# jyjblrd/Low-Cost-Mocap

Hardware: NVIDIA H100
Metric: mocap frame-sets/s (4-cam 640x480 synthetic, blob+epipolar+DLT) (higher is better)
Workload: dtype u8 pixels -> int64 moments -> f64 geometry

## Files before the change

### low-cost-mocap_b200/csrc/api.cu

```cuda
#include <stdarg.h>
#include <stdlib.h>
#include <math.h>
#include <new>
#include "common.cuh"
#include "camera_tables.h"

int blob_kernels_init(mocap_ctx* ctx);
int match_kernels_init(mocap_ctx* ctx);
int fused_kernel_init(mocap_ctx* ctx);
int tma_kernel_init(mocap_ctx* ctx);
int ba_dev_init(mocap_ctx* ctx);

int mocap_fail(mocap_ctx* ctx, int code, const char* fmt, ...) {
    if (ctx) {
        va_list ap;
        va_start(ap, fmt);
        vsnprintf(ctx->err, sizeof(ctx->err), fmt, ap);
        va_end(ap);
    }
    return code;
}

int ensure_scratch(mocap_ctx* ctx, size_t bytes) {
    if (bytes <= ctx->scratch_bytes) return MOCAP_OK;
// ... 28 lines not shown
    cfg->max_blobs = 32;
    cfg->max_segments = 1024;
    cfg->max_roots = 64;
    cfg->max_cands = 8;
    cfg->max_groups = 4096;
}

const char* mocap_last_error(const mocap_ctx* ctx) { return ctx ? ctx->err : "no context"; }

static bool is_pow2(int v) { return v > 0 && (v & (v - 1)) == 0; }

int mocap_create(mocap_ctx** out, const mocap_config* cfg) {
    if (!out || !cfg) return MOCAP_EINVAL;
    *out = nullptr;
    if (cfg->n_cam < 1 || cfg->n_cam > MOCAP_MAX_CAM || cfg->width < 16 || cfg->width % MOCAP_SEG_PX != 0 ||
        cfg->height < 1 || cfg->max_blobs < 1 || cfg->max_blobs > MOCAP_MAX_BLOBS ||
        !is_pow2(cfg->max_segments) || cfg->max_segments < 64 || cfg->max_segments > 4096 ||
        cfg->max_roots < 1 || cfg->max_roots > MOCAP_MAX_ROOTS || cfg->max_cands < 1 || cfg->max_cands > MOCAP_MAX_CANDS ||
        cfg->max_groups < 1 || (long long)cfg->width * cfg->height / MOCAP_SEG_PX > 65535)
        return MOCAP_EINVAL;
    int n_dev = 0;
    if (cudaGetDeviceCount(&n_dev) != cudaSuccess || n_dev <= 0 || cfg->device < 0 || cfg->device >= n_dev) {
        cudaGetLastError();
        return MOCAP_ENODEV;
    }
    cudaDeviceProp prop;
    if (cudaGetDeviceProperties(&prop, cfg->device) != cudaSuccess) return MOCAP_ENODEV;
    if (prop.major != 9 || prop.minor != 0) return MOCAP_ENODEV;
    if (cudaSetDevice(cfg->device) != cudaSuccess) return MOCAP_ENODEV;

    mocap_ctx* ctx = new (std::nothrow) mocap_ctx();
    if (!ctx) return MOCAP_ENOMEM;
    memset(ctx, 0, sizeof(*ctx));
    ctx->cfg = *cfg;
    ctx->num_sms = prop.multiProcessorCount;
    ctx->h_tables.n_cam = cfg->n_cam;
    int st = MOCAP_OK;
    do {
        if (cudaMalloc(&ctx->d_tables, sizeof(CameraTables)) != cudaSuccess) { st = MOCAP_ENOMEM; break; }
        if (cudaStreamCreateWithFlags(&ctx->copy_stream, cudaStreamNonBlocking) != cudaSuccess) { st = MOCAP_ECUDA; break; }
        if (cudaStreamCreateWithFlags(&ctx->copy_stream2, cudaStreamNonBlocking) != cudaSuccess) { st = MOCAP_ECUDA; break; }
        for (int k = 0; k < 2 * 64; ++k)
            if (cudaEventCreate(&ctx->tim_ev[k]) != cudaSuccess) { st = MOCAP_ECUDA; break; }
        if (st) break;
        for (int k = 0; k < 2; ++k) {
            if (cudaEventCreateWithFlags(&ctx->stage_free[k], cudaEventDisableTiming) != cudaSuccess) { st = MOCAP_ECUDA; break; }
            if (cudaEventCreateWithFlags(&ctx->copied[k], cudaEventDisableTiming) != cudaSuccess) { st = MOCAP_ECUDA; break; }
        }
        if (st) break;
        if ((st = blob_kernels_init(ctx)) != MOCAP_OK) break;
        if ((st = match_kernels_init(ctx)) != MOCAP_OK) break;
        {
            const char* mode = getenv("MOCAP_PIPELINE");
            ctx->use_fused = (mode && strcmp(mode, "split") == 0) ? 0 : 1;
            ctx->use_tma = (mode && strcmp(mode, "tma") == 0) ? 1 : 0;
            ctx->use_phased = (mode && strcmp(mode, "phased") == 0) ? 1 : 0;
            ctx->pipeline_auto = (mode && mode[0]) ? 0 : 1;
        }
        {
            void* h = nullptr;
            if (cudaHostAlloc(&h, 2 * sizeof(unsigned long long), cudaHostAllocMapped) != cudaSuccess) { st = MOCAP_ENOMEM; break; }
            memset(h, 0, 2 * sizeof(unsigned long long));
            ctx->h_stat = static_cast<volatile unsigned long long*>(h);
            void* d = nullptr;
            if (cudaHostGetDevicePointer(&d, h, 0) != cudaSuccess) { st = MOCAP_ECUDA; break; }
            ctx->d_stat_host = static_cast<unsigned long long*>(d);
            if (cudaMalloc(&ctx->d_stat_acc, sizeof(unsigned long long)) != cudaSuccess) { st = MOCAP_ENOMEM; break; }
            if (cudaMemset(ctx->d_stat_acc, 0, sizeof(unsigned long long)) != cudaSuccess) { st = MOCAP_ECUDA; break; }
        }
        if ((st = fused_kernel_init(ctx)) != MOCAP_OK) break;
        if ((st = tma_kernel_init(ctx)) != MOCAP_OK) break;
        if ((st = ba_dev_init(ctx)) != MOCAP_OK) break;
        if (ctx->tma_ctas_per_sm < 1) ctx->use_tma = 0;
    } while (0);
    if (st != MOCAP_OK) { mocap_destroy(ctx); return st; }
    *out = ctx;
    return MOCAP_OK;
}

void mocap_destroy(mocap_ctx* ctx) {
    if (!ctx) return;
    cudaSetDevice(ctx->cfg.device);
    cudaDeviceSynchronize();
    cudaFree(ctx->d_tables);
    cudaFree(ctx->d_seg_count); cudaFree(ctx->d_seg_list); cudaFree(ctx->d_worklist); cudaFree(ctx->d_work_count);
    cudaFree(ctx->d_set_worklist); cudaFree(ctx->d_img_done); cudaFree(ctx->d_set_done); cudaFree(ctx->d_unit_counter);
    cudaFree(ctx->d_blob_xy); cudaFree(ctx->d_blob_n); cudaFree(ctx->d_img_flags);
    cudaFree(ctx->d_stage[0]); cudaFree(ctx->d_stage[1]);
    cudaFree(ctx->d_obj); cudaFree(ctx->d_err); cudaFree(ctx->d_nobj); cudaFree(ctx->d_setflags);
    cudaFree(ctx->d_scratch);
    cudaFree(ctx->d_ba_ws);
    cudaFree(ctx->d_match_counter);
    cudaFree(ctx->d_match_items); cudaFree(ctx->d_match_partial); cudaFree(ctx->d_match_range); cudaFree(ctx->d_match_arrive);
    cudaFree(ctx->d_pp_m1); cudaFree(ctx->d_pp_m2); cudaFree(ctx->d_pp_rot);
    cudaFree(ctx->d_stat_acc);
    if (ctx->h_stat) cudaFreeHost(const_cast<unsigned long long*>(ctx->h_stat));
    if (ctx->copy_stream) cudaStreamDestroy(ctx->copy_stream);
    if (ctx->copy_stream2) cudaStreamDestroy(ctx->copy_stream2);
    for (int k = 0; k < 2 * 64; ++k) if (ctx->tim_ev[k]) cudaEventDestroy(ctx->tim_ev[k]);
    for (int k = 0; k < 2; ++k) if (ctx->stage_free[k]) cudaEventDestroy(ctx->stage_free[k]);
    for (int k = 0; k < 2; ++k) if (ctx->copied[k]) cudaEventDestroy(ctx->copied[k]);
    delete ctx;
}

int mocap_set_stream(mocap_ctx* ctx, void* cuda_stream) {
    if (!ctx) return MOCAP_EINVAL;
    ctx->stream = reinterpret_cast<cudaStream_t>(cuda_stream);
    return MOCAP_OK;
}

int mocap_set_cameras(mocap_ctx* ctx, const double* K, const double* R, const double* t) {
    if (!ctx || !K || !R || !t) return MOCAP_EINVAL;
    const int C = ctx->cfg.n_cam;
    CameraTables& T = ctx->h_tables;
    build_camera_tables(T, C, K, R, t);
    CUDA_TRY(ctx, cudaSetDevice(ctx->cfg.device));
    CUDA_TRY(ctx, cudaMemcpyAsync(ctx->d_tables, &T, sizeof(T), cudaMemcpyHostToDevice, ctx->stream));
    CUDA_TRY(ctx, cudaStreamSynchronize(ctx->stream));
    ctx->cameras_set = true;
    return MOCAP_OK;
}

int mocap_set_world_transform(mocap_ctx* ctx, const double* M) {
    if (!ctx) return MOCAP_EINVAL;
    CameraTables& T = ctx->h_tables;
    T.use_world = M ? 1 : 0;
    if (M) memcpy(T.world, M, 16 * sizeof(double));
    CUDA_TRY(ctx, cudaMemcpyAsync(ctx->d_tables, &T, sizeof(T), cudaMemcpyHostToDevice, ctx->stream));
    CUDA_TRY(ctx, cudaStreamSynchronize(ctx->stream));
    return MOCAP_OK;
}

static bool pick_fused(const mocap_ctx* ctx, int channels) {
    if (!ctx->use_fused) return false;
    if (channels != 1 && (ctx->use_tma || ctx->use_phased)) return false;
    if (!ctx->pipeline_auto) return true;
    const unsigned long long blobs = ctx->h_stat[0], images = ctx->h_stat[1];
    if (images == 0) return true;
    return (double)blobs * ctx->cfg.n_cam <= (double)MOCAP_HEAVY_BLOBS_PER_SET * (double)images;
}

static int ensure_images(mocap_ctx* ctx, int n_images) {
    if (n_images <= ctx->cap_images) return MOCAP_OK;
    CUDA_TRY(ctx, cudaStreamSynchronize(ctx->stream));
    cudaFree(ctx->d_seg_count); cudaFree(ctx->d_seg_list); cudaFree(ctx->d_worklist); cudaFree(ctx->d_work_count); cudaFree(ctx->d_set_worklist); cudaFree(ctx->d_img_done); cudaFree(ctx->d_set_done); cudaFree(ctx->d_unit_counter); cudaFree(ctx->d_blob_xy); cudaFree(ctx->d_blob_n); cudaFree(ctx->d_img_flags);
    ctx->d_seg_count = nullptr; ctx->d_seg_list = nullptr; ctx->d_worklist = nullptr; ctx->d_work_count = nullptr; ctx->d_set_worklist = nullptr; ctx->d_img_done = nullptr; ctx->d_set_done = nullptr; ctx->d_unit_counter = nullptr; ctx->d_blob_xy = nullptr; ctx->d_blob_n = nullptr; ctx->d_img_flags = nullptr;
    ctx->cap_images = 0;
    const size_t n = (size_t)n_images;
    CUDA_TRY(ctx, cudaMalloc(&ctx->d_seg_count, n * sizeof(uint32_t)));
    CUDA_TRY(ctx, cudaMalloc(&ctx->d_seg_list, n * ctx->cfg.max_segments * sizeof(uint32_t)));
    CUDA_TRY(ctx, cudaMalloc(&ctx->d_worklist, n * sizeof(uint32_t)));
    CUDA_TRY(ctx, cudaMalloc(&ctx->d_work_count, 4 * sizeof(uint32_t)));
    CUDA_TRY(ctx, cudaMemsetAsync(ctx->d_work_count, 0, 4 * sizeof(uint32_t), ctx->stream));
    CUDA_TRY(ctx, cudaMalloc(&ctx->d_set_worklist, n * sizeof(uint32_t)));
    CUDA_TRY(ctx, cudaMalloc(&ctx->d_img_done, n * sizeof(uint32_t)));
    CUDA_TRY(ctx, cudaMalloc(&ctx->d_set_done, 2 * n * sizeof(uint32_t)));
    CUDA_TRY(ctx, cudaMalloc(&ctx->d_unit_counter, sizeof(unsigned long long)));
    CUDA_TRY(ctx, cudaMemsetAsync(ctx->d_img_done, 0, n * sizeof(uint32_t), ctx->stream));
    CUDA_TRY(ctx, cudaMemsetAsync(ctx->d_set_done, 0, 2 * n * sizeof(uint32_t), ctx->stream));
    CUDA_TRY(ctx, cudaMalloc(&ctx->d_blob_xy, n * ctx->cfg.max_blobs * 2 * sizeof(int32_t)));
    CUDA_TRY(ctx, cudaMalloc(&ctx->d_blob_n, n * sizeof(int32_t)));
    CUDA_TRY(ctx, cudaMalloc(&ctx->d_img_flags, n * sizeof(int32_t)));
    CUDA_TRY(ctx, cudaMemsetAsync(ctx->d_seg_count, 0, n * sizeof(uint32_t), ctx->stream));
    ctx->cap_images = n_images;
    return MOCAP_OK;
}
// ... 239 lines not shown
```

### low-cost-mocap_b200/csrc/ba_dev.cu

```cuda
#include "common.cuh"
#include "ba_device.cuh"

#define BA_THREADS 512

__global__ void __launch_bounds__(BA_THREADS, 1) k_ba_solve(const BAParams P) {
    extern __shared__ __align__(16) unsigned char ba_smem_raw[];
    ba_solve_body(P, ba_smem_raw);
}

__global__ void __launch_bounds__(1024)
k_track_offsets(const int32_t* __restrict__ n_obj, const double* __restrict__ err, int n_sets, int RMAX, double max_err,
                int capacity, int32_t* __restrict__ offs, int32_t* __restrict__ n_points) {
    __shared__ int warp_sum[32];
    __shared__ int carry;
    const int tid = threadIdx.x, lane = tid & 31, wid = tid >> 5;
    if (tid == 0) carry = 0;
    __syncthreads();
    for (int s0 = 0; s0 < n_sets; s0 += blockDim.x) {
        const int s = s0 + tid;
        int kept = 0;
        if (s < n_sets) {
            const int k = min(n_obj[s], RMAX);
            if (max_err > 0.0) { for (int r = 0; r < k; ++r) kept += (err[(size_t)s * RMAX + r] <= max_err) ? 1 : 0; }
            else kept = k;
        }
        int v = kept;
#pragma unroll
        for (int o = 1; o < 32; o <<= 1) { const int u = __shfl_up_sync(0xffffffffu, v, o); if (lane >= o) v += u; }
        if (lane == 31) warp_sum[wid] = v;
        __syncthreads();
        if (wid == 0) {
            int w = lane < (int)(blockDim.x >> 5) ? warp_sum[lane] : 0;
#pragma unroll
            for (int o = 1; o < 32; o <<= 1) { const int u = __shfl_up_sync(0xffffffffu, w, o); if (lane >= o) w += u; }
            warp_sum[lane] = w;
        }
        __syncthreads();
        const int before = carry + (wid > 0 ? warp_sum[wid - 1] : 0) + v - kept;
        if (s < n_sets) offs[s] = before;
        __syncthreads();
        if (tid == (int)blockDim.x - 1) carry = before + kept;
        __syncthreads();
    }
    if (tid == 0) *n_points = carry < capacity ? carry : capacity;
}

__global__ void __launch_bounds__(256)
k_tracks_to_obs(const int32_t* __restrict__ track_xy, const int32_t* __restrict__ n_obj, const double* __restrict__ err,
                const int32_t* __restrict__ offs, int n_sets, int RMAX, int C, double max_err, int capacity,
                double* __restrict__ obs, uint8_t* __restrict__ mask) {
    const long long idx = (long long)blockIdx.x * blockDim.x + threadIdx.x;
    if (idx >= (long long)n_sets * RMAX) return;
    const int s = (int)(idx / RMAX), r = (int)(idx - (long long)s * RMAX);
    if (r >= min(n_obj[s], RMAX)) return;
    int rank = r;
    if (max_err > 0.0) {
        if (!(err[(size_t)s * RMAX + r] <= max_err)) return;
        rank = 0;
        for (int q = 0; q < r; ++q) rank += (err[(size_t)s * RMAX + q] <= max_err) ? 1 : 0;
    }
    const int p = offs[s] + rank;
    if (p >= capacity) return;
    const int32_t* t = track_xy + ((size_t)s * RMAX + r) * C * 2;
    for (int c = 0; c < C; ++c) {
        const int x = t[2 * c], y = t[2 * c + 1];
        const bool seen = x >= 0;
        obs[((size_t)p * C + c) * 2] = seen ? (double)x : 0.0;
        obs[((size_t)p * C + c) * 2 + 1] = seen ? (double)y : 0.0;
        mask[(size_t)p * C + c] = seen ? 1 : 0;
    }
}

int ba_dev_init(mocap_ctx* ctx) {
    const int C = ctx->cfg.n_cam;
    ctx->ba_threads = BA_THREADS;
    ctx->ba_smem = ba_smem_bytes(C, BA_THREADS);
    ctx->ba_grid = 0;
    if (C < 2) return MOCAP_OK;
    if (ctx->ba_smem > 227 * 1024) return MOCAP_OK;
    CUDA_TRY(ctx, cudaFuncSetAttribute(k_ba_solve, cudaFuncAttributeMaxDynamicSharedMemorySize, (int)ctx->ba_smem));
    int per_sm = 0;
    CUDA_TRY(ctx, cudaOccupancyMaxActiveBlocksPerMultiprocessor(&per_sm, k_ba_solve, BA_THREADS, ctx->ba_smem));
    if (per_sm < 1) return MOCAP_OK;
    ctx->ba_grid = ctx->num_sms;
    const char* g = getenv("MOCAP_BA_GRID");
    if (g && atoi(g) > 0 && atoi(g) <= ctx->num_sms * per_sm) ctx->ba_grid = atoi(g);
    return MOCAP_OK;
}

struct BAWorkspace {
    double* X; double* Xnew; uint8_t* valid; double* part; double* fin; double* cpart; unsigned* bar;
    double* Rt_io; int32_t* offs; mocap_ba_report* report;
};

static int ba_workspace(mocap_ctx* ctx, int m_max, int n_sets, BAWorkspace& W, int* pstride_out) {
    const int C = ctx->cfg.n_cam, n = 6 * (C - 1), npair = n * (n + 1) / 2;
    const int pstride = npair + 2 * n + 8, G = ctx->ba_grid;
    auto al = [](size_t b) { return (b + 255) & ~(size_t)255; };
    const size_t sz[] = {al((size_t)m_max * 3 * 8), al((size_t)m_max * 3 * 8), al((size_t)m_max), al((size_t)G * pstride * 8),
                         al((size_t)pstride * 8), al((size_t)2 * G * 4 * 8), al(256), al((size_t)C * 12 * 8),
                         al((size_t)(n_sets > 0 ? n_sets : 1) * 4), al(sizeof(mocap_ba_report))};
    size_t total = 0;
    for (size_t b : sz) total += b;
    if (total > ctx->ba_ws_bytes) {
        CUDA_TRY(ctx, cudaStreamSynchronize(ctx->stream));
        cudaFree(ctx->d_ba_ws);
        ctx->d_ba_ws = nullptr; ctx->ba_ws_bytes = 0;
        CUDA_TRY(ctx, cudaMalloc(&ctx->d_ba_ws, total));
        ctx->ba_ws_bytes = total;
        CUDA_TRY(ctx, cudaMemsetAsync(ctx->d_ba_ws, 0, total, ctx->stream));
    }
    unsigned char* p = static_cast<unsigned char*>(ctx->d_ba_ws);
    W.bar = (unsigned*)p; p += sz[6];
    W.X = (double*)p; p += sz[0]; W.Xnew = (double*)p; p += sz[1]; W.valid = p; p += sz[2];
    W.part = (double*)p; p += sz[3]; W.fin = (double*)p; p += sz[4]; W.cpart = (double*)p; p += sz[5];
    W.Rt_io = (double*)p; p += sz[7]; W.offs = (int32_t*)p; p += sz[8]; W.report = (mocap_ba_report*)p;
    *pstride_out = pstride;
    return MOCAP_OK;
}

extern "C" {

int mocap_set_ba_grid(mocap_ctx* ctx, int n_ctas) {
    if (!ctx) return MOCAP_EINVAL;
    if (ctx->ba_grid < 1) return mocap_fail(ctx, MOCAP_EINVAL, "bundle adjustment is not available for this context (cameras: %d)", ctx->cfg.n_cam);
    if (n_ctas < 0 || n_ctas > ctx->num_sms)
        return mocap_fail(ctx, MOCAP_EINVAL, "mocap_set_ba_grid: %d CTAs asked, 1 .. %d possible (0: default)", n_ctas, ctx->num_sms);
    ctx->ba_grid = n_ctas == 0 ? ctx->num_sms : n_ctas;
    return MOCAP_OK;
}

int mocap_tracks_to_observations_dev(mocap_ctx* ctx, const int32_t* track_xy, const int32_t* n_obj, const double* err,
                                     int n_frame_sets, double max_err, double* obs, uint8_t* mask, int32_t* n_points,
                                     int capacity) {
    if (!ctx) return MOCAP_EINVAL;
    if (!track_xy || !n_obj || !obs || !mask || !n_points || n_frame_sets < 0 || capacity < 1 || (max_err > 0.0 && !err))
        return mocap_fail(ctx, MOCAP_EINVAL, "mocap_tracks_to_observations_dev: bad argument");
    CUDA_TRY(ctx, cudaSetDevice(ctx->cfg.device));
    BAWorkspace W;
    int pstride = 0;
    if (ctx->ba_grid < 1) return mocap_fail(ctx, MOCAP_EINVAL, "bundle adjustment needs at least two cameras");
    int st = ba_workspace(ctx, 1, n_frame_sets, W, &pstride);
    if (st) return st;
    const int RM = ctx->cfg.max_roots, C = ctx->cfg.n_cam;
    k_track_offsets<<<1, 1024, 0, ctx->stream>>>(n_obj, err, n_frame_sets, RM, max_err, capacity, W.offs, n_points);
    CUDA_TRY(ctx, cudaGetLastError());
    const long long total = (long long)n_frame_sets * RM;
    if (total > 0) {
        k_tracks_to_obs<<<(unsigned)((total + 255) / 256), 256, 0, ctx->stream>>>(track_xy, n_obj, err, W.offs, n_frame_sets, RM, C,
                                                                                 max_err, capacity, obs, mask);
        CUDA_TRY(ctx, cudaGetLastError());
    }
    ctx->launches += 2;
    return MOCAP_OK;
}

int mocap_bundle_adjust_dev(mocap_ctx* ctx, const double* obs, const uint8_t* mask, int n_points_max, const int32_t* n_points,
                            double* R, double* t, const mocap_ba_options* opt_in, mocap_ba_report* report) {
    if (!ctx) return MOCAP_EINVAL;
    if (!obs || !mask || !R || !t || n_points_max <= 0) return mocap_fail(ctx, MOCAP_EINVAL, "mocap_bundle_adjust_dev: bad argument");
    if (!ctx->cameras_set) return mocap_fail(ctx, MOCAP_ESTATE, "mocap_set_cameras has not been called (intrinsics are needed)");
    if (ctx->cfg.n_cam < 2) return mocap_fail(ctx, MOCAP_EINVAL, "bundle adjustment needs at least two cameras");
    if (ctx->ba_grid < 1) return mocap_fail(ctx, MOCAP_EINVAL, "k_ba_solve needs %zu bytes of shared memory per CTA for %d cameras", ctx->ba_smem, ctx->cfg.n_cam);
    CUDA_TRY(ctx, cudaSetDevice(ctx->cfg.device));
    mocap_ba_options opt;
    if (opt_in) opt = *opt_in; else mocap_ba_default_options(&opt);
    BAWorkspace W;
    BAParams P;
    memset(&P, 0, sizeof(P));
    int st = ba_workspace(ctx, n_points_max, 0, W, &P.pstride);
    if (st) return st;
    P.tb = ctx->d_tables; P.obs = obs; P.mask = mask; P.m_dev = n_points; P.m_max = n_points_max; P.C = ctx->cfg.n_cam;
    P.R = R; P.t = t;
    P.ftol = opt.ftol; P.xtol = opt.xtol; P.gtol = opt.gtol; P.max_nfev = opt.max_nfev;
    P.jac_mode = opt.jacobian ? 1 : 0; P.prefit = opt.prefit ? 1 : 0; P.prefit_max_iter = opt.prefit_max_iter;
    P.X = W.X; P.Xnew = W.Xnew; P.valid = W.valid; P.part = W.part; P.fin = W.fin; P.cpart = W.cpart; P.bar = W.bar;
    P.report = report;
    void* args[] = {&P};
    CUDA_TRY(ctx, cudaLaunchCooperativeKernel((const void*)k_ba_solve, dim3(ctx->ba_grid), dim3(ctx->ba_threads), args, ctx->ba_smem, ctx->stream));
    ctx->launches += 1;
    return MOCAP_OK;
}

}
```

### low-cost-mocap_b200/csrc/blob_kernels.cu

```cuda
#include "common.cuh"
#include "blob_device.cuh"

template <int UNROLL>
__global__ void __launch_bounds__(256)
k_threshold_segments_c1(const uint4* __restrict__ frames, long long n_seg, int seg_per_image,
                        int max_segments, ThreshConst tc, uint32_t* __restrict__ seg_count,
                        uint32_t* __restrict__ seg_list) {
    const long long stride = (long long)gridDim.x * blockDim.x;
    long long s = (long long)blockIdx.x * blockDim.x + threadIdx.x;
    for (; s < n_seg; s += stride * UNROLL) {
        uint4 v[UNROLL];
#pragma unroll
        for (int u = 0; u < UNROLL; ++u) {
            const long long si = s + stride * u;
            v[u] = (si < n_seg) ? ldg_stream(frames + si) : make_uint4(0, 0, 0, 0);
        }
#pragma unroll
        for (int u = 0; u < UNROLL; ++u) {
            const uint32_t h0 = swar_gt(v[u].x, tc), h1 = swar_gt(v[u].y, tc);
            const uint32_t h2 = swar_gt(v[u].z, tc), h3 = swar_gt(v[u].w, tc);
            if (((h0 | h1 | h2 | h3) & 0x80808080u) == 0) continue;
            const long long si = s + stride * u;
            if (si >= n_seg) continue;
            const uint32_t m = nibble_of(h0) | (nibble_of(h1) << 4) | (nibble_of(h2) << 8) | (nibble_of(h3) << 12);
// ... 76 lines not shown
        const uint32_t* src = seg_list + (size_t)img * E;
        for (int i = lane; i < (int)cnt; i += 32) sm.seg[i] = src[i];
        __syncwarp();
        ok = blob_reduce<32, true, WIDE>(sm, (int)cnt, BLOB_WE, BLOB_WACC, W, H, max_blobs, blob_xy + (size_t)img * max_blobs * 2,
                                   blob_n + img, blob_mom ? blob_mom + (size_t)img * max_blobs * 4 : nullptr, ofl, 0);
    }
    if (lane == 0) {
        if (ok) seg_count[img] = 0;
        else worklist[atomicAdd(work_count, 1u)] = (uint32_t)img;
    }
}

template <int NT, bool WIDE>
__global__ void __launch_bounds__(NT)
k_blob_reduce(uint32_t* __restrict__ seg_count, const uint32_t* __restrict__ seg_list, int E, int W, int H,
              int max_blobs, int32_t* __restrict__ blob_xy, int32_t* __restrict__ blob_n,
              int64_t* __restrict__ blob_mom, int32_t* __restrict__ img_flags,
              const uint32_t* __restrict__ worklist, uint32_t* __restrict__ work_count, uint32_t* __restrict__ done_count,
              int stat_images, unsigned long long* __restrict__ stat_acc, unsigned long long* __restrict__ stat_host) {
    extern __shared__ __align__(16) unsigned char smem_raw[];
    BlobSmem sm = carve_blob_smem(smem_raw, E);
    const unsigned n_work = *work_count;
    for (unsigned w = blockIdx.x; w < n_work; w += gridDim.x) {
        const int img = (int)worklist[w];
        const unsigned cnt = seg_count[img];
        __syncthreads();
        if (threadIdx.x == 0) seg_count[img] = 0;
        int flags = 0;
        int n = (int)cnt;
        if (cnt > (unsigned)E) { flags |= MOCAP_F_SEGMENTS; n = 0; }
        int32_t* ofl = img_flags ? img_flags + img : nullptr;
        if (n == 0) {
            if (threadIdx.x == 0) { blob_n[img] = 0; if (ofl) *ofl = flags; }
            continue;
        }
        const uint32_t* src = seg_list + (size_t)img * E;
        for (int i = threadIdx.x; i < n; i += NT) sm.seg[i] = src[i];
        __syncthreads();
        blob_reduce<NT, false, WIDE>(sm, n, E, MOCAP_ACC_CAP, W, H, max_blobs, blob_xy + (size_t)img * max_blobs * 2, blob_n + img,
                               blob_mom ? blob_mom + (size_t)img * max_blobs * 4 : nullptr, ofl, flags);
        __syncthreads();
    }
    if (stat_host) {
        unsigned long long local = 0;
        for (int i = blockIdx.x * NT + threadIdx.x; i < stat_images; i += gridDim.x * NT) local += (unsigned)__ldcg(blob_n + i);
        for (int o = 16; o; o >>= 1) local += __shfl_xor_sync(0xffffffffu, local, o);
        if ((threadIdx.x & 31) == 0 && local) atomicAdd(stat_acc, local);
        __syncthreads();
    }
    if (threadIdx.x == 0) {
        __threadfence();
        if (atomicAdd(done_count, 1u) == gridDim.x - 1) {
            *work_count = 0; *done_count = 0;
            if (stat_host) {
                __threadfence();
                stat_host[0] = atomicExch(stat_acc, 0ull);
                stat_host[1] = (unsigned long long)stat_images;
            }
        }
    }
}

int launch_detect(mocap_ctx* ctx, const uint8_t* frames, int n_images, int channels, int threshold,
                  int32_t* blob_xy, int32_t* blob_n, int64_t* blob_mom, int32_t* img_flags) {
    const mocap_config& c = ctx->cfg;
    const int seg_per_image = c.width * c.height / MOCAP_SEG_PX;
    const long long n_seg = (long long)n_images * seg_per_image;
    const int E = c.max_segments;
    if (n_images <= 0) return MOCAP_OK;

    if (ctx->timing_on) {
        if (ctx->tim_used == 64) { const int st = timing_flush(ctx); if (st) return st; }
        CUDA_TRY(ctx, cudaEventRecord(ctx->tim_ev[2 * ctx->tim_used], ctx->stream));
    }
    const int threads = 256;
    ThreshConst tc;
    if (threshold < 0) { tc.addc = 0x80808080u; tc.use_and = 0; }
    else if (threshold >= 255) { tc.addc = 0; tc.use_and = 1; }
    else {
        const uint32_t T1 = (uint32_t)threshold + 1u;
        tc.use_and = T1 > 128 ? 1u : 0u;
        tc.addc = (T1 > 128 ? 256u - T1 : 128u - T1) * 0x01010101u;
    }
    const long long cap = (long long)ctx->num_sms * 8;
    if (channels == 1) {
        constexpr int UNROLL = 8;
        long long want = (n_seg + (long long)threads * UNROLL - 1) / ((long long)threads * UNROLL);
        const int grid = (int)(want < cap ? want : cap);
        k_threshold_segments_c1<UNROLL><<<grid, threads, 0, ctx->stream>>>(
            reinterpret_cast<const uint4*>(frames), n_seg, seg_per_image, E, tc, ctx->d_seg_count, ctx->d_seg_list);
    } else {
        constexpr int UNROLL = 2;
        long long want = (n_seg + (long long)threads * UNROLL - 1) / ((long long)threads * UNROLL);
        const int grid = (int)(want < cap ? want : cap);
        k_threshold_segments_c3<UNROLL><<<grid, threads, 0, ctx->stream>>>(
            reinterpret_cast<const uint4*>(frames), n_seg, seg_per_image, E, threshold, tc, ctx->d_seg_count, ctx->d_seg_list);
    }
    CUDA_TRY(ctx, cudaGetLastError());
    if (ctx->timing_on) {
        CUDA_TRY(ctx, cudaEventRecord(ctx->tim_ev[2 * ctx->tim_used + 1], ctx->stream));
        ctx->tim_used += 1;
    }
    constexpr int WPB = 8;
    const long long mx = c.width > c.height ? c.width : c.height;
    const bool wide = 6ll * mx * c.width * c.height >= (1ll << 32);
    if (wide)
        k_blob_reduce_warp<WPB, true><<<(n_images + WPB - 1) / WPB, WPB * 32, 0, ctx->stream>>>(
            ctx->d_seg_count, ctx->d_seg_list, n_images, E, c.width, c.height, c.max_blobs, blob_xy, blob_n, blob_mom, img_flags,
            ctx->d_worklist, ctx->d_work_count);
    else
        k_blob_reduce_warp<WPB, false><<<(n_images + WPB - 1) / WPB, WPB * 32, 0, ctx->stream>>>(
            ctx->d_seg_count, ctx->d_seg_list, n_images, E, c.width, c.height, c.max_blobs, blob_xy, blob_n, blob_mom, img_flags,
            ctx->d_worklist, ctx->d_work_count);
    CUDA_TRY(ctx, cudaGetLastError());
    {
        const int st = launch_blob_fallback(ctx, blob_xy, blob_n, blob_mom, img_flags, n_images);
        if (st) return st;
    }
    ctx->launches += 2;
    return MOCAP_OK;
}

int launch_blob_fallback(mocap_ctx* ctx, int32_t* blob_xy, int32_t* blob_n, int64_t* blob_mom, int32_t* img_flags, int n_images) {
    const mocap_config& c = ctx->cfg;
    constexpr int NT = 128;
    const int E = c.max_segments;
    const size_t smem = blob_reduce_smem_bytes(E);
    const int grid2 = ctx->num_sms;
    const long long mx = c.width > c.height ? c.width : c.height;
    const bool wide = 6ll * mx * c.width * c.height >= (1ll << 32);
    if (wide)
        k_blob_reduce<NT, true><<<grid2, NT, smem, ctx->stream>>>(ctx->d_seg_count, ctx->d_seg_list, E, c.width, c.height,
                                                               c.max_blobs, blob_xy, blob_n, blob_mom, img_flags,
                                                               ctx->d_worklist, ctx->d_work_count, ctx->d_work_count + 1,
                                                               n_images, ctx->d_stat_acc, ctx->pipeline_auto ? ctx->d_stat_host : nullptr);
    else
        k_blob_reduce<NT, false><<<grid2, NT, smem, ctx->stream>>>(ctx->d_seg_count, ctx->d_seg_list, E, c.width, c.height,
                                                                c.max_blobs, blob_xy, blob_n, blob_mom, img_flags,
                                                                ctx->d_worklist, ctx->d_work_count, ctx->d_work_count + 1,
                                                               n_images, ctx->d_stat_acc, ctx->pipeline_auto ? ctx->d_stat_host : nullptr);
    CUDA_TRY(ctx, cudaGetLastError());
    ctx->launches += 1;
    return MOCAP_OK;
}

int timing_flush(mocap_ctx* ctx) {
    for (int i = 0; i < ctx->tim_used; ++i) {
        float ms = 0.f;
        CUDA_TRY(ctx, cudaEventSynchronize(ctx->tim_ev[2 * i + 1]));
        CUDA_TRY(ctx, cudaEventElapsedTime(&ms, ctx->tim_ev[2 * i], ctx->tim_ev[2 * i + 1]));
        ctx->detect_ms_sum += ms;
        ctx->detect_ms_n += 1;
    }
    ctx->tim_used = 0;
    return MOCAP_OK;
}

int blob_kernels_init(mocap_ctx* ctx) {
    const size_t smem = blob_reduce_smem_bytes(ctx->cfg.max_segments);
    CUDA_TRY(ctx, cudaFuncSetAttribute(k_blob_reduce<128, true>, cudaFuncAttributeMaxDynamicSharedMemorySize, (int)smem));
    CUDA_TRY(ctx, cudaFuncSetAttribute(k_blob_reduce<128, false>, cudaFuncAttributeMaxDynamicSharedMemorySize, (int)smem));
    return MOCAP_OK;
}
```

### low-cost-mocap_b200/csrc/common.cuh

```cuda
#pragma once
#include <cuda_runtime.h>
#include <stdint.h>
#include <stdio.h>
#include <string.h>
#include "../../include/mocap_b200.h"

#define MOCAP_MAX_CAM        16
#define MOCAP_MAX_BLOBS      64
#define MOCAP_MAX_ROOTS      128
#define MOCAP_MAX_CANDS      16
#define MOCAP_ACC_CAP        256
#define MOCAP_SEG_PX         16

struct CameraTables {
    double Pkc[MOCAP_MAX_CAM][MOCAP_MAX_CAM][12];
    double F[MOCAP_MAX_CAM][MOCAP_MAX_CAM][9];
    double R[MOCAP_MAX_CAM][9];
    double t[MOCAP_MAX_CAM][3];
    double fx[MOCAP_MAX_CAM], fy[MOCAP_MAX_CAM], cx[MOCAP_MAX_CAM], cy[MOCAP_MAX_CAM];
    double Kmat[MOCAP_MAX_CAM][9];
    double world[16];
    int    use_world;
    int    n_cam;
};

struct mocap_ctx {
    mocap_config cfg;
    cudaStream_t stream;
    cudaStream_t copy_stream;
    cudaStream_t copy_stream2;
    char         err[512];
    bool         cameras_set;
    CameraTables* d_tables;
    CameraTables  h_tables;
    int       cap_images;
    uint32_t* d_seg_count;
    uint32_t* d_seg_list;
    uint32_t* d_worklist;
    uint32_t* d_work_count;
    uint32_t* d_set_worklist;
    uint32_t* d_img_done;
    uint32_t* d_set_done;
    unsigned long long* d_unit_counter;
    int       fused_ctas_per_sm;
    int       tma_ctas_per_sm;
    int       use_tma;
    int       use_phased;
    int       pipeline_auto;
    unsigned long long* d_stat_acc;
    volatile unsigned long long* h_stat;
    unsigned long long* d_stat_host;
    int       use_fused;
    int32_t*  d_blob_xy;
    int32_t*  d_blob_n;
    int32_t*  d_img_flags;
    uint8_t*  d_stage[2];
    size_t    stage_bytes;
    cudaEvent_t stage_free[2]; cudaEvent_t copied[2];
    double*   d_obj; double* d_err; int32_t* d_nobj; int32_t* d_setflags;
    int       cap_sets;
    void*     d_scratch; size_t scratch_bytes;
    void*     d_ba_ws; size_t ba_ws_bytes; int ba_threads; int ba_grid; size_t ba_smem;
    unsigned* d_match_counter; int match_ctas_per_sm;
    void* d_match_items; unsigned long long* d_match_partial; int* d_match_range; unsigned* d_match_arrive;
    int match_chunk, match_item_cap, match_cap_sets;
    const int32_t* img_flags_cur;
    int32_t*  track_xy_cur;
    int16_t*  d_pp_m1; uint16_t* d_pp_m2; int* d_pp_rot; int pp_in_w, pp_in_h;
    uint64_t  launches;
    int       timing_on;
    cudaEvent_t tim_ev[2 * 64];
    int       tim_used;
    double    detect_ms_sum;
    int       detect_ms_n;
    int       num_sms;
};

int mocap_fail(mocap_ctx* ctx, int code, const char* fmt, ...);
#define CUDA_TRY(ctx, call)                                                              \
    do {                                                                                 \
        cudaError_t e__ = (call);                                                        \
        if (e__ != cudaSuccess)                                                          \
            return mocap_fail((ctx), MOCAP_ECUDA, "%s failed: %s (%s:%d)", #call,        \
                              cudaGetErrorString(e__), __FILE__, __LINE__);              \
    } while (0)

int launch_detect(mocap_ctx* ctx, const uint8_t* frames, int n_images, int channels, int threshold,
                  int32_t* blob_xy, int32_t* blob_n, int64_t* blob_mom, int32_t* img_flags);
int launch_match(mocap_ctx* ctx, const int32_t* blob_xy, const int32_t* blob_n, int n_sets,
                 double* obj, double* err, int32_t* n_obj, int32_t* set_flags, int32_t* chosen);
int launch_triangulate(mocap_ctx* ctx, const double* obs, const uint8_t* mask, int n_points,
                       const double* X_in, double* X, double* err, uint8_t* valid);
int ensure_scratch(mocap_ctx* ctx, size_t bytes);
int launch_locate(mocap_ctx* ctx, const double* obj, const double* err, const int32_t* n_obj, int n_sets,
                  int max_objects, double* out, int32_t* drone_index, int32_t* n_out);
int launch_blob_fallback(mocap_ctx* ctx, int32_t* blob_xy, int32_t* blob_n, int64_t* blob_mom, int32_t* img_flags, int n_images);
#define MOCAP_HEAVY_BLOBS_PER_SET 48
#define MOCAP_MATCH_CHUNK 512
int launch_match_list(mocap_ctx* ctx, const int32_t* blob_xy, const int32_t* blob_n, const uint32_t* set_list, uint32_t* set_count,
                      int n_sets_max, double* obj, double* err, int32_t* n_obj, int32_t* set_flags);
int launch_pipeline_tma(mocap_ctx* ctx, const uint8_t* frames, int n_sets, int threshold,
                        double* obj, double* err, int32_t* n_obj, int32_t* set_flags);
int launch_pipeline_fused(mocap_ctx* ctx, const uint8_t* frames, int n_sets, int threshold,
                          double* obj, double* err, int32_t* n_obj, int32_t* set_flags, int channels = 1);
int timing_flush(mocap_ctx* ctx);
```

### low-cost-mocap_b200/csrc/match_kernels.cu

```cuda
#include <cstdlib>
#include <cstring>
#include "common.cuh"
#include "geom.cuh"
#include "match_device.cuh"

__global__ void __launch_bounds__(128)
k_match_triangulate(const CameraTables* __restrict__ tb, const int32_t* blob_xy, const int32_t* blob_n,
                    const uint32_t* __restrict__ set_list, uint32_t* set_count, MatchSplit sp,
                    int n_sets, int C, int MB, int RMAX, int KC,
                    uint32_t GMAX, double* __restrict__ obj, double* __restrict__ err_out,
                    int32_t* __restrict__ n_obj, int32_t* __restrict__ set_flags, int32_t* __restrict__ chosen,
                    int32_t* __restrict__ track_xy, const int32_t* __restrict__ img_flags) {
    extern __shared__ __align__(16) unsigned char smem_raw[];
    const int warps = blockDim.x >> 5;
    const int wid = threadIdx.x >> 5, lane = threadIdx.x & 31;
    WarpState ws = carve_warp_state(smem_raw + warp_state_bytes(RMAX, C, KC, MB) * wid, RMAX, C, KC, MB);
    if (set_list) {
        const unsigned n_work = *set_count;
        for (unsigned w = blockIdx.x * warps + wid; w < n_work; w += gridDim.x * warps) {
            const int set = (int)set_list[w];
            match_triangulate_warp(tb, ws, blob_xy + (size_t)set * C * MB * 2, blob_n + (size_t)set * C, set, lane,
                                   C, MB, RMAX, KC, GMAX, obj, err_out, n_obj, set_flags, chosen, track_xy,
                                   img_flags ? img_flags + (size_t)set * C : nullptr);
            __syncwarp();
// ... 22 lines not shown
__global__ void __launch_bounds__(128)
k_triangulate_points(const CameraTables* __restrict__ tb, const double* __restrict__ obs,
                     const uint8_t* __restrict__ mask, int n_points, int C,
                     const double* __restrict__ X_in, double* __restrict__ X_out,
                     double* __restrict__ err_out, uint8_t* __restrict__ valid) {
    const int f = blockIdx.x * blockDim.x + threadIdx.x;
    if (f >= n_points) return;
    const double* o = obs + (size_t)f * C * 2;
    const uint8_t* m = mask + (size_t)f * C;
    int nv = 0;
    for (int c = 0; c < C; ++c) nv += m[c] ? 1 : 0;
    if (nv <= 1) {
        if (valid) valid[f] = 0;
        if (X_out) { X_out[3 * f] = X_out[3 * f + 1] = X_out[3 * f + 2] = nan(""); }
        if (err_out) err_out[f] = nan("");
        return;
    }
    double X[3];
    if (X_in) { X[0] = X_in[3 * f]; X[1] = X_in[3 * f + 1]; X[2] = X_in[3 * f + 2]; }
    else {
        Sym4 B;
        sym4_zero(B);
        int k = 0;
        for (int c = 0; c < C; ++c)
            if (m[c]) { dlt_add_view(B, tb->Pkc[k][c], o[2 * c], o[2 * c + 1]); ++k; }
        dlt_solve(B, X);
    }
    if (X_out) { X_out[3 * f] = X[0]; X_out[3 * f + 1] = X[1]; X_out[3 * f + 2] = X[2]; }
    if (valid) valid[f] = 1;
    if (err_out) {
        double sq[2 * MOCAP_MAX_CAM];
        int k = 0;
        for (int c = 0; c < C; ++c)
            if (m[c]) {
                float u, v;
                project_like_cv(tb->R[c], tb->t[c], tb->fx[k], tb->fy[k], tb->cx[k], tb->cy[k], X, u, v);
                const double dx = DSUB(o[2 * c], (double)u), dy = DSUB(o[2 * c + 1], (double)v);
                sq[2 * k] = DMUL(dx, dx); sq[2 * k + 1] = DMUL(dy, dy);
                ++k;
            }
        err_out[f] = mean_like_numpy(sq, 2 * nv, false);
    }
}

static int ensure_match_split(mocap_ctx* ctx, int n_sets) {
    long long want = (long long)n_sets * 4 > 4096 ? (long long)n_sets * 4 : 4096;
    const long long per_item = (long long)ctx->cfg.max_roots * MATCH_PARTIAL_WORDS * (long long)sizeof(unsigned long long);
    if (want * per_item > (512ll << 20)) want = (512ll << 20) / per_item;
    const int want_items = (int)want;
    if (n_sets <= ctx->match_cap_sets && want_items <= ctx->match_item_cap) return MOCAP_OK;
    CUDA_TRY(ctx, cudaStreamSynchronize(ctx->stream));
    cudaFree(ctx->d_match_items); cudaFree(ctx->d_match_partial); cudaFree(ctx->d_match_range); cudaFree(ctx->d_match_arrive);
    ctx->d_match_items = nullptr; ctx->d_match_partial = nullptr; ctx->d_match_range = nullptr; ctx->d_match_arrive = nullptr;
    ctx->match_cap_sets = 0; ctx->match_item_cap = 0;
    CUDA_TRY(ctx, cudaMalloc(&ctx->d_match_items, (size_t)want_items * sizeof(MatchItem)));
    CUDA_TRY(ctx, cudaMalloc(&ctx->d_match_partial, (size_t)want_items * ctx->cfg.max_roots * MATCH_PARTIAL_WORDS * sizeof(unsigned long long)));
    CUDA_TRY(ctx, cudaMalloc(&ctx->d_match_range, (size_t)want_items * 2 * sizeof(int)));
    CUDA_TRY(ctx, cudaMalloc(&ctx->d_match_arrive, (size_t)n_sets * sizeof(unsigned)));
    CUDA_TRY(ctx, cudaMemsetAsync(ctx->d_match_arrive, 0, (size_t)n_sets * sizeof(unsigned), ctx->stream));
    ctx->match_cap_sets = n_sets; ctx->match_item_cap = want_items;
    return MOCAP_OK;
}

int launch_match(mocap_ctx* ctx, const int32_t* blob_xy, const int32_t* blob_n, int n_sets,
                 double* obj, double* err, int32_t* n_obj, int32_t* set_flags, int32_t* chosen) {
    if (n_sets <= 0) return MOCAP_OK;
    const mocap_config& c = ctx->cfg;
    const int warps = 4;
    const size_t smem = match_smem_bytes(c, warps);
    const int full = ctx->num_sms * ctx->match_ctas_per_sm;
    int grid = (n_sets + warps - 1) / warps;
    if (grid > full) grid = full;
    MatchSplit sp;
    memset(&sp, 0, sizeof(sp));
    sp.counters = ctx->d_match_counter;
    if (ctx->match_chunk > 0) {
        const int st = ensure_match_split(ctx, n_sets);
        if (st) return st;
        sp.items = static_cast<MatchItem*>(ctx->d_match_items);
        sp.partial = ctx->d_match_partial; sp.range = ctx->d_match_range; sp.arrive = ctx->d_match_arrive;
        sp.chunk = (uint32_t)ctx->match_chunk; sp.item_cap = (uint32_t)ctx->match_item_cap;
    }
    CUDA_TRY(ctx, cudaMemsetAsync(ctx->d_match_counter, 0, 4 * sizeof(unsigned), ctx->stream));
    k_match_triangulate<<<grid, warps * 32, smem, ctx->stream>>>(ctx->d_tables, blob_xy, blob_n, nullptr, nullptr, sp, n_sets, c.n_cam,
                                                                 c.max_blobs, c.max_roots, c.max_cands,
                                                                 (uint32_t)c.max_groups, obj, err, n_obj, set_flags, chosen, ctx->track_xy_cur, ctx->img_flags_cur);
    CUDA_TRY(ctx, cudaGetLastError());
    ctx->launches += 1;
    if (sp.items) {
        k_match_chunks<<<full, warps * 32, smem, ctx->stream>>>(ctx->d_tables, blob_xy, blob_n, sp, c.n_cam, c.max_blobs, c.max_roots, c.max_cands,
                                                                (uint32_t)c.max_groups, obj, err, n_obj, set_flags, chosen, ctx->track_xy_cur, ctx->img_flags_cur);
        CUDA_TRY(ctx, cudaGetLastError());
        ctx->launches += 1;
    }
    return MOCAP_OK;
}

int launch_match_list(mocap_ctx* ctx, const int32_t* blob_xy, const int32_t* blob_n, const uint32_t* set_list, uint32_t* set_count,
                      int n_sets_max, double* obj, double* err, int32_t* n_obj, int32_t* set_flags) {
    const mocap_config& c = ctx->cfg;
    const int warps = 4;
    const size_t smem = match_smem_bytes(c, warps);
    int grid = (n_sets_max + warps - 1) / warps;
    if (grid > ctx->num_sms) grid = ctx->num_sms;
    MatchSplit none;
    memset(&none, 0, sizeof(none));
    k_match_triangulate<<<grid, warps * 32, smem, ctx->stream>>>(ctx->d_tables, blob_xy, blob_n, set_list, set_count, none, n_sets_max, c.n_cam,
                                                                 c.max_blobs, c.max_roots, c.max_cands, (uint32_t)c.max_groups,
                                                                 obj, err, n_obj, set_flags, nullptr, ctx->track_xy_cur, ctx->d_img_flags);
    CUDA_TRY(ctx, cudaGetLastError());
    ctx->launches += 1;
    return MOCAP_OK;
}

int launch_triangulate(mocap_ctx* ctx, const double* obs, const uint8_t* mask, int n_points,
                       const double* X_in, double* X, double* err, uint8_t* valid) {
    if (n_points <= 0) return MOCAP_OK;
    const int threads = 128;
    k_triangulate_points<<<(n_points + threads - 1) / threads, threads, 0, ctx->stream>>>(
        ctx->d_tables, obs, mask, n_points, ctx->cfg.n_cam, X_in, X, err, valid);
    CUDA_TRY(ctx, cudaGetLastError());
    ctx->launches += 1;
    return MOCAP_OK;
}

int match_kernels_init(mocap_ctx* ctx) {
    const size_t smem = match_smem_bytes(ctx->cfg, 4);
    if (smem > 200 * 1024) return mocap_fail(ctx, MOCAP_EINVAL, "matcher state needs %zu bytes of shared memory per CTA; lower max_roots/max_cands", smem);
    CUDA_TRY(ctx, cudaFuncSetAttribute(k_match_triangulate, cudaFuncAttributeMaxDynamicSharedMemorySize, (int)smem));
    int per_sm = 0;
    CUDA_TRY(ctx, cudaOccupancyMaxActiveBlocksPerMultiprocessor(&per_sm, k_match_triangulate, 128, smem));
    ctx->match_ctas_per_sm = per_sm > 0 ? per_sm : 1;
    CUDA_TRY(ctx, cudaFuncSetAttribute(k_match_chunks, cudaFuncAttributeMaxDynamicSharedMemorySize, (int)smem));
    CUDA_TRY(ctx, cudaMalloc(&ctx->d_match_counter, 4 * sizeof(unsigned)));
    const char* ch = getenv("MOCAP_MATCH_CHUNK");
    int chunk = ch && ch[0] ? atoi(ch) : MOCAP_MATCH_CHUNK;
    if (chunk < 0) chunk = 0;
    ctx->match_chunk = (chunk + 31) / 32 * 32;
    return MOCAP_OK;
}
```

Before: 2.307 million.

## Shrink BA solver footprint and co-schedule detect/match kernels beside in-flight BA

The bundle-adjustment cooperative kernel drops from 512 to 384 threads with a 128-register cap and a max-shared carveout. A global registry of contexts with a completion event now reports when a BA solve is still running on the device. While one is, the threshold, reduce and match kernels launch with a max-shared carveout, and the threshold grids are sized to the registers the BA kernel leaves free, so both can share SMs. The frame-set throughput path likely runs no BA, which leaves only a host-side mutex and event query per launch, while the smaller BA block may change solver speed or spill registers.

```diff
diff --git a/low-cost-mocap_b200/csrc/api.cu b/low-cost-mocap_b200/csrc/api.cu
--- a/low-cost-mocap_b200/csrc/api.cu
+++ b/low-cost-mocap_b200/csrc/api.cu
@@ -134,6 +134,7 @@
     if (!ctx) return;
     cudaSetDevice(ctx->cfg.device);
     cudaDeviceSynchronize();
+    ba_dev_release(ctx);
     cudaFree(ctx->d_tables);
     cudaFree(ctx->d_seg_count); cudaFree(ctx->d_seg_list); cudaFree(ctx->d_worklist); cudaFree(ctx->d_work_count);
     cudaFree(ctx->d_set_worklist); cudaFree(ctx->d_img_done); cudaFree(ctx->d_set_done); cudaFree(ctx->d_unit_counter);
diff --git a/low-cost-mocap_b200/csrc/ba_dev.cu b/low-cost-mocap_b200/csrc/ba_dev.cu
--- a/low-cost-mocap_b200/csrc/ba_dev.cu
+++ b/low-cost-mocap_b200/csrc/ba_dev.cu
@@ -1,9 +1,10 @@
+#include <algorithm>
+#include <mutex>
+#include <vector>
 #include "common.cuh"
 #include "ba_device.cuh"
 
-#define BA_THREADS 512
-
-__global__ void __launch_bounds__(BA_THREADS, 1) k_ba_solve(const BAParams P) {
+__global__ void __maxnreg__(BA_REGS) k_ba_solve(const BAParams P) {
     extern __shared__ __align__(16) unsigned char ba_smem_raw[];
     ba_solve_body(P, ba_smem_raw);
 }
@@ -71,14 +72,33 @@
     }
 }
 
+static std::mutex g_ba_mu;
+static std::vector<mocap_ctx*> g_ba_ctx;
+
+bool ba_solve_in_flight(int device) {
+    std::lock_guard<std::mutex> lock(g_ba_mu);
+    for (mocap_ctx* c : g_ba_ctx)
+        if (c->cfg.device == device && cudaEventQuery(c->ba_done) == cudaErrorNotReady) return true;
+    return false;
+}
+
+void ba_dev_release(mocap_ctx* ctx) {
+    std::lock_guard<std::mutex> lock(g_ba_mu);
+    g_ba_ctx.erase(std::remove(g_ba_ctx.begin(), g_ba_ctx.end(), ctx), g_ba_ctx.end());
+    if (ctx->ba_done) cudaEventDestroy(ctx->ba_done);
+    ctx->ba_done = nullptr;
+}
+
 int ba_dev_init(mocap_ctx* ctx) {
     const int C = ctx->cfg.n_cam;
     ctx->ba_threads = BA_THREADS;
     ctx->ba_smem = ba_smem_bytes(C, BA_THREADS);
     ctx->ba_grid = 0;
     if (C < 2) return MOCAP_OK;
+    CUDA_TRY(ctx, cudaEventCreateWithFlags(&ctx->ba_done, cudaEventDisableTiming));
     if (ctx->ba_smem > 227 * 1024) return MOCAP_OK;
     CUDA_TRY(ctx, cudaFuncSetAttribute(k_ba_solve, cudaFuncAttributeMaxDynamicSharedMemorySize, (int)ctx->ba_smem));
+    CUDA_TRY(ctx, cudaFuncSetAttribute(k_ba_solve, cudaFuncAttributePreferredSharedMemoryCarveout, (int)cudaSharedmemCarveoutMaxShared));
     int per_sm = 0;
     CUDA_TRY(ctx, cudaOccupancyMaxActiveBlocksPerMultiprocessor(&per_sm, k_ba_solve, BA_THREADS, ctx->ba_smem));
     if (per_sm < 1) return MOCAP_OK;
@@ -178,6 +198,11 @@
     P.report = report;
     void* args[] = {&P};
     CUDA_TRY(ctx, cudaLaunchCooperativeKernel((const void*)k_ba_solve, dim3(ctx->ba_grid), dim3(ctx->ba_threads), args, ctx->ba_smem, ctx->stream));
+    CUDA_TRY(ctx, cudaEventRecord(ctx->ba_done, ctx->stream));
+    {
+        std::lock_guard<std::mutex> lock(g_ba_mu);
+        if (std::find(g_ba_ctx.begin(), g_ba_ctx.end(), ctx) == g_ba_ctx.end()) g_ba_ctx.push_back(ctx);
+    }
     ctx->launches += 1;
     return MOCAP_OK;
 }
diff --git a/low-cost-mocap_b200/csrc/blob_kernels.cu b/low-cost-mocap_b200/csrc/blob_kernels.cu
--- a/low-cost-mocap_b200/csrc/blob_kernels.cu
+++ b/low-cost-mocap_b200/csrc/blob_kernels.cu
@@ -182,19 +182,21 @@
         tc.use_and = T1 > 128 ? 1u : 0u;
         tc.addc = (T1 > 128 ? 256u - T1 : 128u - T1) * 0x01010101u;
     }
-    const long long cap = (long long)ctx->num_sms * 8;
+    const bool beside_ba = ba_solve_in_flight(c.device);
     if (channels == 1) {
         constexpr int UNROLL = 8;
+        const long long cap = (long long)ctx->num_sms * (beside_ba ? ctx->stream_ctas_c1 : 8);
         long long want = (n_seg + (long long)threads * UNROLL - 1) / ((long long)threads * UNROLL);
         const int grid = (int)(want < cap ? want : cap);
-        k_threshold_segments_c1<UNROLL><<<grid, threads, 0, ctx->stream>>>(
-            reinterpret_cast<const uint4*>(frames), n_seg, seg_per_image, E, tc, ctx->d_seg_count, ctx->d_seg_list);
+        CUDA_TRY(ctx, launch_beside_ba(beside_ba, k_threshold_segments_c1<UNROLL>, dim3(grid), dim3(threads), 0, ctx->stream,
+            reinterpret_cast<const uint4*>(frames), n_seg, seg_per_image, E, tc, ctx->d_seg_count, ctx->d_seg_list));
     } else {
         constexpr int UNROLL = 2;
+        const long long cap = (long long)ctx->num_sms * (beside_ba ? ctx->stream_ctas_c3 : 8);
         long long want = (n_seg + (long long)threads * UNROLL - 1) / ((long long)threads * UNROLL);
         const int grid = (int)(want < cap ? want : cap);
-        k_threshold_segments_c3<UNROLL><<<grid, threads, 0, ctx->stream>>>(
-            reinterpret_cast<const uint4*>(frames), n_seg, seg_per_image, E, threshold, tc, ctx->d_seg_count, ctx->d_seg_list);
+        CUDA_TRY(ctx, launch_beside_ba(beside_ba, k_threshold_segments_c3<UNROLL>, dim3(grid), dim3(threads), 0, ctx->stream,
+            reinterpret_cast<const uint4*>(frames), n_seg, seg_per_image, E, threshold, tc, ctx->d_seg_count, ctx->d_seg_list));
     }
     CUDA_TRY(ctx, cudaGetLastError());
     if (ctx->timing_on) {
@@ -205,13 +207,13 @@
     const long long mx = c.width > c.height ? c.width : c.height;
     const bool wide = 6ll * mx * c.width * c.height >= (1ll << 32);
     if (wide)
-        k_blob_reduce_warp<WPB, true><<<(n_images + WPB - 1) / WPB, WPB * 32, 0, ctx->stream>>>(
+        CUDA_TRY(ctx, launch_beside_ba(beside_ba, k_blob_reduce_warp<WPB, true>, dim3((n_images + WPB - 1) / WPB), dim3(WPB * 32), 0, ctx->stream,
             ctx->d_seg_count, ctx->d_seg_list, n_images, E, c.width, c.height, c.max_blobs, blob_xy, blob_n, blob_mom, img_flags,
-            ctx->d_worklist, ctx->d_work_count);
+            ctx->d_worklist, ctx->d_work_count));
     else
-        k_blob_reduce_warp<WPB, false><<<(n_images + WPB - 1) / WPB, WPB * 32, 0, ctx->stream>>>(
+        CUDA_TRY(ctx, launch_beside_ba(beside_ba, k_blob_reduce_warp<WPB, false>, dim3((n_images + WPB - 1) / WPB), dim3(WPB * 32), 0, ctx->stream,
             ctx->d_seg_count, ctx->d_seg_list, n_images, E, c.width, c.height, c.max_blobs, blob_xy, blob_n, blob_mom, img_flags,
-            ctx->d_worklist, ctx->d_work_count);
+            ctx->d_worklist, ctx->d_work_count));
     CUDA_TRY(ctx, cudaGetLastError());
     {
         const int st = launch_blob_fallback(ctx, blob_xy, blob_n, blob_mom, img_flags, n_images);
@@ -229,16 +231,17 @@
     const int grid2 = ctx->num_sms;
     const long long mx = c.width > c.height ? c.width : c.height;
     const bool wide = 6ll * mx * c.width * c.height >= (1ll << 32);
+    const bool beside_ba = ba_solve_in_flight(c.device);
     if (wide)
-        k_blob_reduce<NT, true><<<grid2, NT, smem, ctx->stream>>>(ctx->d_seg_count, ctx->d_seg_list, E, c.width, c.height,
-                                                               c.max_blobs, blob_xy, blob_n, blob_mom, img_flags,
-                                                               ctx->d_worklist, ctx->d_work_count, ctx->d_work_count + 1,
-                                                               n_images, ctx->d_stat_acc, ctx->pipeline_auto ? ctx->d_stat_host : nullptr);
+        CUDA_TRY(ctx, launch_beside_ba(beside_ba, k_blob_reduce<NT, true>, dim3(grid2), dim3(NT), smem, ctx->stream,
+            ctx->d_seg_count, ctx->d_seg_list, E, c.width, c.height, c.max_blobs, blob_xy, blob_n, blob_mom, img_flags,
+            ctx->d_worklist, ctx->d_work_count, ctx->d_work_count + 1, n_images, ctx->d_stat_acc,
+            ctx->pipeline_auto ? ctx->d_stat_host : nullptr));
     else
-        k_blob_reduce<NT, false><<<grid2, NT, smem, ctx->stream>>>(ctx->d_seg_count, ctx->d_seg_list, E, c.width, c.height,
-                                                                c.max_blobs, blob_xy, blob_n, blob_mom, img_flags,
-                                                                ctx->d_worklist, ctx->d_work_count, ctx->d_work_count + 1,
-                                                               n_images, ctx->d_stat_acc, ctx->pipeline_auto ? ctx->d_stat_host : nullptr);
+        CUDA_TRY(ctx, launch_beside_ba(beside_ba, k_blob_reduce<NT, false>, dim3(grid2), dim3(NT), smem, ctx->stream,
+            ctx->d_seg_count, ctx->d_seg_list, E, c.width, c.height, c.max_blobs, blob_xy, blob_n, blob_mom, img_flags,
+            ctx->d_worklist, ctx->d_work_count, ctx->d_work_count + 1, n_images, ctx->d_stat_acc,
+            ctx->pipeline_auto ? ctx->d_stat_host : nullptr));
     CUDA_TRY(ctx, cudaGetLastError());
     ctx->launches += 1;
     return MOCAP_OK;
@@ -260,5 +263,12 @@
     const size_t smem = blob_reduce_smem_bytes(ctx->cfg.max_segments);
     CUDA_TRY(ctx, cudaFuncSetAttribute(k_blob_reduce<128, true>, cudaFuncAttributeMaxDynamicSharedMemorySize, (int)smem));
     CUDA_TRY(ctx, cudaFuncSetAttribute(k_blob_reduce<128, false>, cudaFuncAttributeMaxDynamicSharedMemorySize, (int)smem));
-    return MOCAP_OK;
-}
+    int regs = 0, per_sm = 0;
+    CUDA_TRY(ctx, cudaDeviceGetAttribute(&regs, cudaDevAttrMaxRegistersPerMultiprocessor, ctx->cfg.device));
+    const int left = regs - BA_THREADS * BA_REGS;
+    CUDA_TRY(ctx, cudaOccupancyMaxActiveBlocksPerMultiprocessor(&per_sm, k_threshold_segments_c1<8>, 256, 0));
+    ctx->stream_ctas_c1 = per_sm * left / regs > 0 ? per_sm * left / regs : 1;
+    CUDA_TRY(ctx, cudaOccupancyMaxActiveBlocksPerMultiprocessor(&per_sm, k_threshold_segments_c3<2>, 256, 0));
+    ctx->stream_ctas_c3 = per_sm * left / regs > 0 ? per_sm * left / regs : 1;
+    return MOCAP_OK;
+}
diff --git a/low-cost-mocap_b200/csrc/common.cuh b/low-cost-mocap_b200/csrc/common.cuh
--- a/low-cost-mocap_b200/csrc/common.cuh
+++ b/low-cost-mocap_b200/csrc/common.cuh
@@ -61,7 +61,9 @@
     int       cap_sets;
     void*     d_scratch; size_t scratch_bytes;
     void*     d_ba_ws; size_t ba_ws_bytes; int ba_threads; int ba_grid; size_t ba_smem;
+    cudaEvent_t ba_done;
     unsigned* d_match_counter; int match_ctas_per_sm;
+    int stream_ctas_c1, stream_ctas_c3;
     void* d_match_items; unsigned long long* d_match_partial; int* d_match_range; unsigned* d_match_arrive;
     int match_chunk, match_item_cap, match_cap_sets;
     const int32_t* img_flags_cur;
@@ -85,6 +87,26 @@
                               cudaGetErrorString(e__), __FILE__, __LINE__);              \
     } while (0)
 
+#define BA_THREADS 384
+#define BA_REGS 128
+bool ba_solve_in_flight(int device);
+void ba_dev_release(mocap_ctx* ctx);
+
+#ifdef __CUDACC__
+#include <utility>
+template <typename... Exp, typename... Act>
+static inline cudaError_t launch_beside_ba(bool beside_ba, void (*kernel)(Exp...), dim3 grid, dim3 block, size_t smem,
+                                           cudaStream_t stream, Act&&... args) {
+    cudaLaunchAttribute attr;
+    attr.id = cudaLaunchAttributePreferredSharedMemoryCarveout;
+    attr.val.sharedMemCarveout = cudaSharedmemCarveoutMaxShared;
+    cudaLaunchConfig_t cfg = {};
+    cfg.gridDim = grid; cfg.blockDim = block; cfg.dynamicSmemBytes = smem; cfg.stream = stream;
+    cfg.attrs = &attr; cfg.numAttrs = beside_ba ? 1 : 0;
+    return cudaLaunchKernelEx(&cfg, kernel, std::forward<Act>(args)...);
+}
+#endif
+
 int launch_detect(mocap_ctx* ctx, const uint8_t* frames, int n_images, int channels, int threshold,
                   int32_t* blob_xy, int32_t* blob_n, int64_t* blob_mom, int32_t* img_flags);
 int launch_match(mocap_ctx* ctx, const int32_t* blob_xy, const int32_t* blob_n, int n_sets,
diff --git a/low-cost-mocap_b200/csrc/match_kernels.cu b/low-cost-mocap_b200/csrc/match_kernels.cu
--- a/low-cost-mocap_b200/csrc/match_kernels.cu
+++ b/low-cost-mocap_b200/csrc/match_kernels.cu
@@ -128,14 +128,16 @@
         sp.chunk = (uint32_t)ctx->match_chunk; sp.item_cap = (uint32_t)ctx->match_item_cap;
     }
     CUDA_TRY(ctx, cudaMemsetAsync(ctx->d_match_counter, 0, 4 * sizeof(unsigned), ctx->stream));
-    k_match_triangulate<<<grid, warps * 32, smem, ctx->stream>>>(ctx->d_tables, blob_xy, blob_n, nullptr, nullptr, sp, n_sets, c.n_cam,
-                                                                 c.max_blobs, c.max_roots, c.max_cands,
-                                                                 (uint32_t)c.max_groups, obj, err, n_obj, set_flags, chosen, ctx->track_xy_cur, ctx->img_flags_cur);
+    const bool beside_ba = ba_solve_in_flight(c.device);
+    CUDA_TRY(ctx, launch_beside_ba(beside_ba, k_match_triangulate, dim3(grid), dim3(warps * 32), smem, ctx->stream, ctx->d_tables, blob_xy, blob_n,
+                                   nullptr, nullptr, sp, n_sets, c.n_cam, c.max_blobs, c.max_roots, c.max_cands, (uint32_t)c.max_groups,
+                                   obj, err, n_obj, set_flags, chosen, ctx->track_xy_cur, ctx->img_flags_cur));
     CUDA_TRY(ctx, cudaGetLastError());
     ctx->launches += 1;
     if (sp.items) {
-        k_match_chunks<<<full, warps * 32, smem, ctx->stream>>>(ctx->d_tables, blob_xy, blob_n, sp, c.n_cam, c.max_blobs, c.max_roots, c.max_cands,
-                                                                (uint32_t)c.max_groups, obj, err, n_obj, set_flags, chosen, ctx->track_xy_cur, ctx->img_flags_cur);
+        CUDA_TRY(ctx, launch_beside_ba(beside_ba, k_match_chunks, dim3(full), dim3(warps * 32), smem, ctx->stream, ctx->d_tables, blob_xy, blob_n,
+                                       sp, c.n_cam, c.max_blobs, c.max_roots, c.max_cands, (uint32_t)c.max_groups,
+                                       obj, err, n_obj, set_flags, chosen, ctx->track_xy_cur, ctx->img_flags_cur));
         CUDA_TRY(ctx, cudaGetLastError());
         ctx->launches += 1;
     }
```

New measurement: 2.307 million (median of 6 runs). About the same (+0.0%).
